# Kmatsuo57/cell-image-analysis

Hardware: NVIDIA B200
Metric: cells scored/sec (crop+resize+CAE+SVM) (higher is better)
Workload: dtype f16 tensor cores (CAE, PCA, SVM cross term: fp16 hi+lo operands, fp32 accumulate) / f64 norms and sums

## Files before the change

cell-image-analysis_b200/csrc/api.cu:

```cuda
#include "common.cuh"

#include <cmath>
#include <cstdlib>
#include <cstring>
#include <new>

#define CIA_VERSION 100

static int bad_handle() { return CIA_E_ARG; }

template <typename T>
static int upload(cia_ctx* h, T** dst, const T* src, size_t n) {
    cudaFree(*dst); *dst = nullptr;
    CIA_CUDA(cudaMalloc((void**)dst, n * sizeof(T)));
    CIA_CUDA(cudaMemcpy(*dst, src, n * sizeof(T), cudaMemcpyHostToDevice));
    return CIA_OK;
}

extern "C" {

int cia_version(void) { return CIA_VERSION; }

void cia_default_params(cia_params* p) {
    if (!p) return;
    p->border_margin = 10;
    p->area_min = 200;
    p->area_max = 8000;
    p->ecc_max = 0.95;
    p->mean_min = 0.5;
    p->std_min = 0.1;
    p->clip_limit = 0.02;
    p->intensity_inv = 1.0 / 65535.0;
}

int cia_create(int device, cia_handle* out) {
    if (!out) return CIA_E_ARG;
    *out = nullptr;
    cia_ctx* h = new (std::nothrow) cia_ctx();
    if (!h) return CIA_E_ARG;
    h->device = device;
    cudaError_t e = cudaSetDevice(device);
    if (e != cudaSuccess) { delete h; return CIA_E_CUDA; }
    cudaDeviceProp prop;
    if (cudaGetDeviceProperties(&prop, device) == cudaSuccess) { h->num_sms = prop.multiProcessorCount; h->max_smem_optin = (int)prop.sharedMemPerBlockOptin; }
    if (cudaMalloc(&h->status_dev, sizeof(int32_t)) != cudaSuccess ||
        cudaMemset(h->status_dev, 0, sizeof(int32_t)) != cudaSuccess ||
        cudaMallocHost(&h->status_host, sizeof(int32_t)) != cudaSuccess ||
        cudaEventCreateWithFlags(&h->ev, cudaEventDisableTiming) != cudaSuccess ||
        cudaEventCreateWithFlags(&h->ev_fork, cudaEventDisableTiming) != cudaSuccess ||
        cudaEventCreateWithFlags(&h->ev_join, cudaEventDisableTiming) != cudaSuccess ||
        cudaStreamCreateWithFlags(&h->side, cudaStreamNonBlocking) != cudaSuccess) {
        delete h;
        return CIA_E_CUDA;
    }
    if (const char* e = getenv("CIA_CAE_CHUNK")) { const int v = atoi(e); if (v > 0) h->cae_pass_cells = v; }
    if (const char* e = getenv("CIA_L1_DEBIAS")) h->cae_debias[0] = (float)atof(e);
    if (const char* e = getenv("CIA_L2_DEBIAS")) h->cae_debias[1] = (float)atof(e);
    if (const char* e = getenv("CIA_L3_DEBIAS")) h->cae_debias[2] = (float)atof(e);
    if (const char* e = getenv("CIA_SVM_KERNEL")) h->svm_kernel = atoi(e) ? 1 : 0;
    if (const char* e = getenv("CIA_PCA_KERNEL")) h->pca_kernel = atoi(e) ? 1 : 0;
    *out = h;
    return CIA_OK;
}

int cia_set_option(cia_handle h, const char* name, double value) {
    if (!h) return bad_handle();
    if (!name) { h->err = "cia_set_option: null name"; return CIA_E_ARG; }
    const std::string n(name);
    if (n == "cae_pass_cells") {
        if (!(value >= 1 && value <= 1 << 20)) { h->err = "cia_set_option: cae_pass_cells must be in [1, 2^20]"; return CIA_E_ARG; }
        h->cae_pass_cells = (int)value;
    } else if (n == "cae_l1_debias" || n == "cae_l2_debias" || n == "cae_l3_debias") {
        if (!(value >= 0 && value <= 64)) { h->err = "cia_set_option: debias must be in [0, 64] (units of 2^-24)"; return CIA_E_ARG; }
        h->cae_debias[n[5] - '1'] = (float)value;
    } else if (n == "svm_kernel") {
        if (value != 0 && value != 1) { h->err = "cia_set_option: svm_kernel is 0 (fp64 DMMA) or 1 (tcgen05)"; return CIA_E_ARG; }
        h->svm_kernel = (int)value;
    } else if (n == "pca_kernel") {
        if (value != 0 && value != 1) { h->err = "cia_set_option: pca_kernel is 0 (fp64 DMMA) or 1 (tcgen05)"; return CIA_E_ARG; }
        h->pca_kernel = (int)value;
    } else if (n == "svm_refine") {
        h->svm_refine = value != 0;
    } else if (n == "seg_conv_tma") {
        h->seg_conv_tma = value != 0;
    } else if (n == "seg_pool_out") {
        h->seg_pool_out = value != 0;
    } else if (n == "seg_fuse_first") {
        h->seg_fuse_first = value != 0;
    } else if (n == "seg_conv_ws") {
        if (value != 0 && value != 1 && value != 2) { h->err = "cia_set_option: seg_conv_ws is 0 (off), 1 (where it pays) or 2 (every layer)"; return CIA_E_ARG; }
        h->seg_conv_ws = (int)value;
    } else {
        h->err = "cia_set_option: unknown option '" + n + "'";
        return CIA_E_ARG;
    }
    return CIA_OK;
}

static void free_cae(CaeWeights& w) {
    for (int i = 0; i < CAE_NCONV; ++i) {
        cudaFree(w.kernel[i]); cudaFree(w.bias[i]); cudaFree(w.bn_scale[i]); cudaFree(w.bn_shift[i]);
        w.kernel[i] = w.bias[i] = w.bn_scale[i] = w.bn_shift[i] = nullptr;
    }
    for (int i = 0; i < CAE_NCONV; ++i)
        for (int j = 0; j < 2; ++j) { cudaFree(w.tc_w[i][j]); w.tc_w[i][j] = nullptr; }
    cudaFree(w.tc_w7); w.tc_w7 = nullptr;
    w.tc_ready = false;
    w.loaded = false;
}

int cia_destroy(cia_handle h) {
    if (!h) return bad_handle();
    cudaSetDevice(h->device);
    cudaDeviceSynchronize();
    free_cae(h->cae[0]); free_cae(h->cae[1]);
    k_seg_free(h);
    cudaFree(h->sp.center); cudaFree(h->sp.scale); cudaFree(h->sp.rscale); cudaFree(h->sp.comp_t); cudaFree(h->sp.comp_pad); cudaFree(h->sp.offset); cudaFree(h->sp.tc_img); cudaFree(h->sp.tc_par);
    for (int i = 0; i < 2; ++i) { cudaFree(h->svm[i].sv_t); cudaFree(h->svm[i].coef); cudaFree(h->svm[i].sv_pad); cudaFree(h->svm[i].gsn);
                                  cudaFree(h->svm[i].tc_hi); cudaFree(h->svm[i].tc_lo); cudaFree(h->svm[i].tc_gcol); }
    Workspace* ws[] = {&h->ws_flags, &h->ws_act, &h->ws_crop_scratch, &h->ws_pipe, &h->ws_feat,
                       &h->ws_misc, &h->ws_stage, &h->ws_svm, &h->ws_fit};
    for (Workspace* w : ws) cudaFree(w->p);
    cudaFree(h->status_dev);
    cudaFreeHost(h->status_host);
    if (h->ev) cudaEventDestroy(h->ev);
    if (h->ev_fork) cudaEventDestroy(h->ev_fork);
    if (h->ev_join) cudaEventDestroy(h->ev_join);
// ... 512 lines not shown
```

cell-image-analysis_b200/csrc/cae_tc.cu:

```cuda
#include "common.cuh"
#include "tc_ptx.cuh"

#include <cuda.h>
#include <cuda_fp16.h>

#include <cmath>

namespace {

constexpr int TCT = 256;
enum { EPI_POOL = 0, EPI_PLAIN = 2, EPI_FINAL = 3, EPI_PHASE = 4 };

using namespace tcptx;

#ifdef CIA_LANE0_ISSUE
#define ISSUE_WARP(cond) (lane == 0 && (cond))
#define ISSUE_BEGIN {
#define ISSUE_END }
#else
#define ISSUE_WARP(cond) (cond)
#define ISSUE_BEGIN if (elect_one()) {
#define ISSUE_END } __syncwarp();
#endif
#ifdef CIA_SPIN_WAIT
// ... 963 lines not shown
                                    fadd2(acc[2 * hp + p2][k8 * 8 + k], acc[2 * hp + p2][k8 * 8 + k + 1],
                                          v[p2][k8][k], v[p2][k8][k + 1]);
                    }
                    DBG_T(e5);
                    DBG_ADD(e_add, e3, e5);
                    ++it;
                }
                DBG_T(e6);
                constexpr int RO = R / 2;
                const int Y = ROWPAIR ? r >> 4 : r >> 3, X = 8 * sub + (r & 7);
#pragma unroll
                for (int k8 = 0; k8 < CW / 8; ++k8) {
                    const int c0 = cq * CW + k8 * 8;
                    float o[8];
#pragma unroll
                    for (int k = 0; k < 8; ++k) {
                        const float b = __ldg(bias + c0 + k), sc = __ldg(bn_s + c0 + k), sh = __ldg(bn_t + c0 + k);
                        float m = acc[0][k8 * 8 + k];
#pragma unroll
                        for (int ph = 1; ph < NT; ++ph) m = fmaxf(m, acc[ph][k8 * 8 + k]);
                        if (ROWPAIR) m = fmaxf(m, __shfl_xor_sync(0xffffffffu, m, 8));
                        o[k] = pooled_act(m, inv_scale, invd, b, sc, sh);
                    }
                    if (ROWPAIR && (r & 8)) continue;
                    const size_t off = ((((size_t)cell * (COUT / 8) + c0 / 8) * RO + Y) * RO + X) * 8;
                    split_store8(o, out_hi + off, out_lo ? out_lo + off : nullptr);
                    if (feat) {
                        float4* f = reinterpret_cast<float4*>(feat + (size_t)cell * (RO * RO * COUT) +
                                                             (size_t)(Y * RO + X) * COUT + c0);
                        f[0] = make_float4(o[0], o[1], o[2], o[3]);
                        f[1] = make_float4(o[4], o[5], o[6], o[7]);
                    }
                }
                DBG_T(e7);
                DBG_ADD(e_final, e6, e7);
            }
        }
#ifdef CIA_ACC_TIMING
        if (tid == 0) {
            atomicAdd(&g_acc_dbg[0], (unsigned long long)e_stage);
            atomicAdd(&g_acc_dbg[1], (unsigned long long)e_full);
            atomicAdd(&g_acc_dbg[2], (unsigned long long)e_ld);
            atomicAdd(&g_acc_dbg[3], (unsigned long long)e_add);
            atomicAdd(&g_acc_dbg[4], (unsigned long long)e_final);
            atomicAdd(&g_acc_dbg[5], (unsigned long long)e_units);
        }
#endif
    }
    tc_fence_before();
    __syncthreads();
    if (warp == 0) tmem_dealloc(tmem_base, TMEM_COLS);
}

template <int G, int VAR = 0>
__global__ void __launch_bounds__(ACC_THREADS, 1)
conv_tc_l2_stack_kernel(const __grid_constant__ CUtensorMap tm_hi, const __grid_constant__ CUtensorMap tm_lo,
                        const uint4* __restrict__ w_hi, const uint4* __restrict__ w_lo, float inv_scale, float invd,
                        const float* __restrict__ bias, const float* __restrict__ bn_s,
                        const float* __restrict__ bn_t, __half* __restrict__ out_hi, __half* __restrict__ out_lo,
                        float* __restrict__ feat, int n_cells, const int32_t* __restrict__ n_dev, int cell0,
                        int chunk_cells) {
    constexpr int CIN = 32, COUT = 64, R = 32;
    using C = Acc2Cfg<CIN, COUT, R>;
    constexpr int NGRP = (9 + G - 1) / G;
    constexpr int CW = COUT / 4;
    constexpr int TILE_COLS = 2 * COUT;
    constexpr int WS_B = 2 * C::W_B;
    extern __shared__ __align__(1024) unsigned char smem[];
    __shared__ __align__(8) uint64_t full_bar[4], empty_bar[4], ready_bar[2];
    __shared__ uint32_t tmem_base_s;

    const int tid = threadIdx.x, warp = tid >> 5, lane = tid & 31;
    unsigned char* const w_s = smem + C::HALVES * C::BUF_B;

    int n = dev_count(n_cells, n_dev) - cell0;
    if (n > chunk_cells) n = chunk_cells;
    if (n <= 0) return;
    const int n_units = n;

    if (warp == 0) tmem_alloc(&tmem_base_s, 512);
    if (tid == 32) {
        for (int t = 0; t < 4; ++t) { mbar_init(&full_bar[t], 1); mbar_init(&empty_bar[t], ACC_EPI_WARPS); }
        mbar_init(&ready_bar[0], 1); mbar_init(&ready_bar[1], 1);
        fence_barrier_init();
    }
    for (int i = tid; i < WS_B / 16; i += ACC_THREADS) {
        const int tc = i / (2 * COUT), row = i - tc * (2 * COUT);
        reinterpret_cast<uint4*>(w_s)[i] = row < COUT ? __ldg(w_hi + tc * COUT + row) : __ldg(w_lo + tc * COUT + row - COUT);
    }
    fence_async_smem();
    tc_fence_before();
    __syncthreads();
    tc_fence_after();
    const uint32_t tmem_base = tmem_base_s;
    const uint32_t sbase = smem_u32(smem);
    constexpr uint32_t IDESC64 = make_idesc(128, COUT), IDESC128 = make_idesc(128, 2 * COUT);

    if (warp >= ACC_EPI_WARPS) {
        if (warp - ACC_EPI_WARPS < 4) {
            const int t = warp - ACC_EPI_WARPS, py = t >> 1, px = t & 1;
            const uint64_t b_s0 = make_smem_desc(smem_u32(w_s), 2 * COUT * 16, 128);
            const uint64_t b_l0 = b_s0 + (uint64_t)((COUT * 16) >> 4);
            uint64_t dxo[3];
#pragma unroll
            for (int dx = 0; dx < 3; ++dx) dxo[dx] = (uint64_t)((((px + dx) & 1) * C::PAR_B + ((px + dx) >> 1) * 16) >> 4);
            const uint32_t d_main = tmem_base + (uint32_t)(t * TILE_COLS), d_cross = d_main + COUT;
// ... 604 lines not shown
                                              w.bn_scale[layer], w.bn_shift[layer], out_hi, out_lo, feat, n, n_dev,
                                              cell0, chunk);
    CIA_LAUNCH_CHECK();
    acc_timing_dump("acc", CIN, COUT, R, G, s);
    return CIA_OK;
}

typedef CUresult (*TensorMapEncodeFn)(CUtensorMap*, CUtensorMapDataType, cuuint32_t, void*, const cuuint64_t*,
                                      const cuuint64_t*, const cuuint32_t*, const cuuint32_t*, CUtensorMapInterleave,
                                      CUtensorMapSwizzle, CUtensorMapL2promotion, CUtensorMapFloatOOBfill);

static int encode_act_map(cia_ctx* h, CUtensorMap* tm, const __half* base, int nch, int r, int cells, int box_x,
                          int box_y) {
    static TensorMapEncodeFn encode = [] {
        void* fn = nullptr;
        cudaDriverEntryPointQueryResult q;
        if (cudaGetDriverEntryPoint("cuTensorMapEncodeTiled", &fn, cudaEnableDefault, &q) != cudaSuccess) fn = nullptr;
        return (TensorMapEncodeFn)fn;
    }();
    if (!encode) { h->err = "cuTensorMapEncodeTiled is not available from this driver"; return CIA_E_UNSUPPORTED; }
    const cuuint64_t dims[5] = {8, (cuuint64_t)r, (cuuint64_t)r, (cuuint64_t)nch, (cuuint64_t)cells};
    const cuuint64_t strides[4] = {16, (cuuint64_t)16 * r, (cuuint64_t)16 * r * r, (cuuint64_t)16 * r * r * nch};
    const cuuint32_t box[5] = {8, (cuuint32_t)box_x, (cuuint32_t)box_y, (cuuint32_t)nch, 1};
    const cuuint32_t estr[5] = {1, 2, 1, 1, 1};
    const CUresult rc = encode(tm, CU_TENSOR_MAP_DATA_TYPE_FLOAT16, 5, (void*)base, dims, strides, box, estr,
                               CU_TENSOR_MAP_INTERLEAVE_NONE, CU_TENSOR_MAP_SWIZZLE_NONE,
                               CU_TENSOR_MAP_L2_PROMOTION_L2_128B, CU_TENSOR_MAP_FLOAT_OOB_FILL_NONE);
    if (rc != CUDA_SUCCESS) { h->err = "cuTensorMapEncodeTiled failed"; return CIA_E_CUDA; }
    return CIA_OK;
}

template <int CIN, int COUT, int R, int G>
int launch_tc_acc2(cia_ctx* h, const CaeWeights& w, int layer, const __half* in_hi, const __half* in_lo,
                   int buf_cells, __half* out_hi, __half* out_lo, float* feat, int n, const int32_t* n_dev,
                   int cell0, int chunk, cudaStream_t s) {
    using C = Acc2Cfg<CIN, COUT, R>;
    static_assert(C::SMEM_B + 1280 <= 227 * 1024, "double-buffered blocks do not fit in shared memory");
    auto kern = conv_tc_acc2_kernel<CIN, COUT, R, G>;
    if (first_use(h, (const void*)kern))
        CIA_CUDA(cudaFuncSetAttribute(kern, cudaFuncAttributeMaxDynamicSharedMemorySize, C::SMEM_B));
    CUtensorMap tm_hi, tm_lo;
    int rc;
    if ((rc = encode_act_map(h, &tm_hi, in_hi, C::NCH, C::R, buf_cells, C::BOX_X, C::FILL_ROWS))) return rc;
    if ((rc = encode_act_map(h, &tm_lo, in_lo, C::NCH, C::R, buf_cells, C::BOX_X, C::FILL_ROWS))) return rc;
    int grid = chunk;
    if (grid > h->num_sms) grid = h->num_sms;
    kern<<<grid, ACC_THREADS, C::SMEM_B, s>>>(tm_hi, tm_lo, (const uint4*)w.tc_w[layer][0],
                                              (const uint4*)w.tc_w[layer][1], w.tc_inv_scale[layer],
                                              w.tc_inv_scale[layer] * acc_debias(h, layer), w.bias[layer],
                                              w.bn_scale[layer], w.bn_shift[layer], out_hi, out_lo, feat, n, n_dev,
                                              cell0, chunk);
    CIA_LAUNCH_CHECK();
    acc_timing_dump("acc2", CIN, COUT, R, G, s);
    return CIA_OK;
}

template <int G, int VAR = 0>
int launch_l2_stack(cia_ctx* h, const CaeWeights& w, const __half* in_hi, const __half* in_lo, int buf_cells,
                    __half* out_hi, __half* out_lo, float* feat, int n, const int32_t* n_dev, int cell0, int chunk,
                    cudaStream_t s) {
    using C = Acc2Cfg<32, 64, 32>;
    auto kern = conv_tc_l2_stack_kernel<G, VAR>;
    if (first_use(h, (const void*)kern))
        CIA_CUDA(cudaFuncSetAttribute(kern, cudaFuncAttributeMaxDynamicSharedMemorySize, C::SMEM_B));
    CUtensorMap tm_hi, tm_lo;
    int rc;
    if ((rc = encode_act_map(h, &tm_hi, in_hi, C::NCH, C::R, buf_cells, C::BOX_X, C::FILL_ROWS))) return rc;
    if ((rc = encode_act_map(h, &tm_lo, in_lo, C::NCH, C::R, buf_cells, C::BOX_X, C::FILL_ROWS))) return rc;
    int grid = chunk;
    if (grid > h->num_sms) grid = h->num_sms;
    kern<<<grid, ACC_THREADS, C::SMEM_B, s>>>(tm_hi, tm_lo, (const uint4*)w.tc_w[1][0], (const uint4*)w.tc_w[1][1],
                                              w.tc_inv_scale[1], w.tc_inv_scale[1] * acc_debias(h, 1), w.bias[1],
                                              w.bn_scale[1], w.bn_shift[1], out_hi, out_lo, feat, n, n_dev, cell0, chunk);
    CIA_LAUNCH_CHECK();
    return CIA_OK;
}

static void pack_image(const std::vector<float>& w , int taps, int cin, int N,
                       int n_real, int sw, std::vector<__half>& hi, std::vector<__half>& lo,
                       const float* colsign = nullptr) {
    const int nch = cin / 8;
    hi.assign((size_t)taps * nch * N * 8, __float2half_rn(0.f));
    lo = hi;
    const float sc = std::ldexp(1.f, sw);
    for (int tap = 0; tap < taps; ++tap)
        for (int c = 0; c < cin; ++c)
            for (int nn = 0; nn < n_real; ++nn) {
                const float v = w[((size_t)tap * cin + c) * n_real + nn] * sc * (colsign ? colsign[nn] : 1.f);
                const __half hv = __float2half_rn(v);
                const size_t idx = (((size_t)tap * nch + c / 8) * N + nn) * 8 + (c % 8);
                hi[idx] = hv;
                lo[idx] = __float2half_rn(v - __half2float(hv));
            }
}

static int scale_exp(const std::vector<float>& w) {
    float m = 0.f;
    for (float v : w) m = std::fmax(m, std::fabs(v));
    if (!(m > 0.f)) return 0;
    int e;
    std::frexp(m, &e);
    return 2 - e;
}

}

// ... 121 lines not shown
        A2f = (float*)h->ws_act.p;
    }
    __half* A1h = (__half*)h->ws_misc.p;
    __half* A1l = A1h + CH * a1;
    __half* A2h = A1l + CH * a1;
    __half* A2l = A2h + CH * a2;
    __half* A3h = A2l + CH * a2;
    __half* A4u = A3h + CH * a3;
    __half* A5u = A4u + CH * a4u;
    __half* A6 = A5u + CH * a5u;
    CIA_CUDA(cudaMemsetAsync(mse, 0, (size_t)n * sizeof(float), s));
    CIA_CUDA(cudaMemsetAsync(mae, 0, (size_t)n * sizeof(float), s));
    const bool side_encoder = features && !tc_feat && !l3_exact;
    if (side_encoder) {
        CIA_CUDA(cudaEventRecord(h->ev_fork, s));
        CIA_CUDA(cudaStreamWaitEvent(h->side, h->ev_fork, 0));
        rc = k_encoder_fp32(h, sep ? h->cae[1] : h->cae[0], crops, n, n_dev, features, h->side);
        if (rc) return rc;
        CIA_CUDA(cudaEventRecord(h->ev_join, h->side));
    }
    for (int c0 = 0; c0 < n; c0 += CH) {
        const int chunk = (n - c0) < CH ? (n - c0) : CH;
        __half* a1h = A1h - (size_t)c0 * a1; __half* a1l = A1l - (size_t)c0 * a1;
        __half* a2h = A2h - (size_t)c0 * a2; __half* a2l = A2l - (size_t)c0 * a2;
        __half* a3h = A3h - (size_t)c0 * a3; __half* a4 = A4u - (size_t)c0 * a4u;
        __half* a5 = A5u - (size_t)c0 * a5u; __half* a6p = A6 - (size_t)c0 * a6;
        float* feat = tc_feat ? features : nullptr;
        int grid1 = chunk * 4;
        if (grid1 > h->num_sms * 8) grid1 = h->num_sms * 8;
        const int pass = c0 / CH;
        if (h->layer_ev && pass < CIA_LAYER_PASSES) h->layer_passes = pass + 1;
#define CIA_LMARK(i) do { if (h->layer_ev && pass < CIA_LAYER_PASSES) CIA_CUDA(cudaEventRecord(h->layer_ev[pass * CIA_LAYER_MARKS + (i)], s)); } while (0)
        CIA_LMARK(0);
        if (tc_feat || l3_exact) {
            static const int l1_tc = [] { const char* e = getenv("CIA_L1_KERNEL"); return e ? atoi(e) : 1; }();
            const float l1_debias = h->cae_debias[0] * 5.9604645e-8f;
            if (l1_tc) {
                if (first_use(h, (const void*)conv1_tc_split_kernel))
                    CIA_CUDA(cudaFuncSetAttribute(conv1_tc_split_kernel, cudaFuncAttributeMaxDynamicSharedMemorySize, l1tc::SMEM_B));
                int gridt = chunk * 8;
                if (gridt > h->num_sms * 2) gridt = h->num_sms * 2;
                conv1_tc_split_kernel<<<gridt, l1tc::NT, l1tc::SMEM_B, s>>>(crops, (const uint4*)ae.tc_w[0][0], ae.tc_inv_scale[0],
                                                                            l1_debias, ae.bias[0], ae.bn_scale[0], ae.bn_shift[0],
                                                                            a1h, a1l, n, n_dev, c0, chunk);
            } else {
                conv1_fp32_planar_kernel<<<grid1, 256, 0, s>>>(crops, ae.kernel[0], ae.bias[0], ae.bn_scale[0],
                                                               ae.bn_shift[0], a1h, a1l, n, n_dev, c0, chunk);
            }
            CIA_LAUNCH_CHECK();
            CIA_LMARK(1);
            float* a2f = l3_exact ? A2f - (size_t)c0 * (16 * 16 * 64) : nullptr;
            static const int l2_g = [] { const char* e = getenv("CIA_L2_TAPS_PER_FLUSH"); return e ? atoi(e) : 3; }();
            static const int l2_stack = [] { const char* e = getenv("CIA_L2_STACK"); return e ? atoi(e) : 0; }();
            if (l2_stack == 2 && l2_g == 3) rc = launch_l2_stack<3, 1>(h, ae, A1h, A1l, CH, a2h, a2l, a2f, n, n_dev, c0, chunk, s);
            else if (l2_stack == 3 && l2_g == 3) rc = launch_l2_stack<3, 2>(h, ae, A1h, A1l, CH, a2h, a2l, a2f, n, n_dev, c0, chunk, s);
            else if (l2_stack && l2_g == 3) rc = launch_l2_stack<3>(h, ae, A1h, A1l, CH, a2h, a2l, a2f, n, n_dev, c0, chunk, s);
            else if (l2_g == 0) rc = launch_tc_acc<32, 64, 32, 1>(h, ae, 1, a1h, a1l, a2h, a2l, a2f, n, n_dev, c0, chunk, s);
            else if (l2_g == 1) rc = launch_tc_acc2<32, 64, 32, 1>(h, ae, 1, A1h, A1l, CH, a2h, a2l, a2f, n, n_dev, c0, chunk, s);
            else if (l2_g == 9) rc = launch_tc_acc2<32, 64, 32, 9>(h, ae, 1, A1h, A1l, CH, a2h, a2l, a2f, n, n_dev, c0, chunk, s);
            else if (l2_g == 2) rc = launch_tc_acc2<32, 64, 32, 2>(h, ae, 1, A1h, A1l, CH, a2h, a2l, a2f, n, n_dev, c0, chunk, s);
            else rc = launch_tc_acc2<32, 64, 32, 3>(h, ae, 1, A1h, A1l, CH, a2h, a2l, a2f, n, n_dev, c0, chunk, s);
            if (rc) return rc;
            CIA_LMARK(2);
            if (l3_exact) {
                if ((rc = launch_tc<64, 32, 16, EPI_POOL, 1>(h, ae, 2, a2h, nullptr, a3h, nullptr, nullptr, nullptr, nullptr, nullptr, n, n_dev, c0, chunk, s))) return rc;
                if (features && (rc = k_conv3_fp32(h, ae, a2f, n, n_dev, features, c0, chunk, s))) return rc;
            } else {
                static const int l3_tma = [] { const char* e = getenv("CIA_L3_KERNEL"); return e ? atoi(e) : 0; }();
                static const int l3_g = [] { const char* e = getenv("CIA_L3_TAPS_PER_FLUSH"); return e ? atoi(e) : 1; }();
                if (l3_tma) rc = launch_tc_acc2<64, 32, 16, 1>(h, ae, 2, A2h, A2l, CH, a3h, nullptr, feat, n, n_dev, c0, chunk, s);
                else if (l3_g == 3) rc = launch_tc_acc<64, 32, 16, 3>(h, ae, 2, a2h, a2l, a3h, nullptr, feat, n, n_dev, c0, chunk, s);
                else rc = launch_tc_acc<64, 32, 16, 1>(h, ae, 2, a2h, a2l, a3h, nullptr, feat, n, n_dev, c0, chunk, s);
                if (rc) return rc;
            }
        } else {
            conv1_fp32_planar_kernel<<<grid1, 256, 0, s>>>(crops, ae.kernel[0], ae.bias[0], ae.bn_scale[0],
                                                           ae.bn_shift[0], a1h, nullptr, n, n_dev, c0, chunk);
            CIA_LAUNCH_CHECK();
            CIA_LMARK(1);
            if ((rc = launch_tc<32, 64, 32, EPI_POOL, 1>(h, ae, 1, a1h, nullptr, a2h, nullptr, nullptr, nullptr, nullptr, nullptr, n, n_dev, c0, chunk, s))) return rc;
            CIA_LMARK(2);
            if ((rc = launch_tc<64, 32, 16, EPI_POOL, 1>(h, ae, 2, a2h, nullptr, a3h, nullptr, nullptr, nullptr, nullptr, nullptr, n, n_dev, c0, chunk, s))) return rc;
        }
        CIA_LMARK(3);
        if ((rc = launch_tc<32, 32, 8, EPI_PLAIN, 1>(h, ae, 3, a3h, nullptr, a4, nullptr, nullptr, nullptr, nullptr, nullptr, n, n_dev, c0, chunk, s))) return rc;
        CIA_LMARK(4);
        if ((rc = launch_tc<32, 64, 16, EPI_PLAIN, 1, true>(h, ae, 4, a4, nullptr, a5, nullptr, nullptr, nullptr, nullptr, nullptr, n, n_dev, c0, chunk, s))) return rc;
        CIA_LMARK(5);
        if ((rc = launch_tc<64, 128, 16, EPI_PHASE, 1>(h, ae, 5, a5, nullptr, a6p, nullptr, nullptr, nullptr, nullptr, nullptr, n, n_dev, c0, chunk, s))) return rc;
        CIA_LMARK(6);
        static const int l7_tapsum = [] { const char* e = getenv("CIA_L7_KERNEL"); return e ? atoi(e) : 1; }();
        if (l7_tapsum) {
            if (first_use(h, (const void*)final_tapsum_kernel))
                CIA_CUDA(cudaFuncSetAttribute(final_tapsum_kernel, cudaFuncAttributeMaxDynamicSharedMemorySize, l7::SMEM_B));
            int g7 = chunk < h->num_sms ? chunk : h->num_sms;
            final_tapsum_kernel<<<g7, l7::NT, l7::SMEM_B, s>>>(a6p, (const uint4*)ae.tc_w7, ae.tc_inv_scale[6], ae.bias[6],
                                                              crops, mse, mae, n, n_dev, c0, chunk);
            CIA_LAUNCH_CHECK();
        } else if ((rc = launch_tc<32, 16, 32, EPI_FINAL, 1>(h, ae, 6, a6p, nullptr, nullptr, nullptr, nullptr, crops, mse, mae, n, n_dev, c0, chunk, s))) return rc;
        CIA_LMARK(7);
#undef CIA_LMARK
    }
    if (side_encoder) CIA_CUDA(cudaStreamWaitEvent(s, h->ev_join, 0));
    return CIA_OK;
}
```

cell-image-analysis_b200/csrc/common.cuh:

```cuda
#pragma once
#include <cuda_runtime.h>
#include <stdint.h>
#include <stdio.h>
#include <set>
#include <string>
#include <vector>

#include "../../include/cia.h"

#define CIA_NUM_SMS_DEFAULT 148

#define CAE_NCONV 7
static const int kCaeCin[CAE_NCONV]  = {1, 32, 64, 32, 32, 64, 32};
static const int kCaeCout[CAE_NCONV] = {32, 64, 32, 32, 64, 32, 1};

struct CaeWeights {
    bool loaded = false;
    int n_conv = 0;
    float* kernel[CAE_NCONV] = {};
    float* bias[CAE_NCONV] = {};
    float* bn_scale[CAE_NCONV] = {};
    float* bn_shift[CAE_NCONV] = {};
    void* tc_w[CAE_NCONV][2] = {};
    void* tc_w7 = nullptr;
// ... 19 lines not shown

struct ScalerPca {
    bool loaded = false;
    int F = 0, C = 0;
    int center_is_f32 = 1, f32_flow = 1, has_center = 0, has_scale = 0;
    double* center = nullptr;
    double* scale = nullptr;
    double* rscale = nullptr;
    bool rscale_ok = false;
    double* comp_t = nullptr;
    double* comp_pad = nullptr;
    int CP = 0;
    double* offset = nullptr;
    void* tc_img = nullptr;
    void* tc_par = nullptr;
    int tc_ew = 0;
    bool tc_ok = false;
};

struct Workspace {
    void* p = nullptr;
    size_t cap = 0;
};

struct SegModel;

struct cia_ctx {
    int device = 0;
    SegModel* seg = nullptr;
    int num_sms = CIA_NUM_SMS_DEFAULT;
    int max_smem_optin = 227 * 1024;
    std::string err;
    CaeWeights cae[2];
    ScalerPca sp;
    SvmModel svm[2];
    int32_t* status_dev = nullptr;
    int32_t* status_host = nullptr;
    int64_t launches = 0;
    std::set<const void*> attr_done;
    Workspace ws_flags, ws_act, ws_crop_scratch, ws_pipe, ws_feat, ws_misc, ws_stage, ws_svm;
    Workspace ws_fit;
    cudaEvent_t ev = nullptr;
    cudaStream_t side = nullptr;
    cudaEvent_t ev_fork = nullptr, ev_join = nullptr;
    std::vector<cudaEvent_t> prof_ev;
    std::vector<cudaEvent_t> prof_layer_ev;
    std::vector<int> prof_layer_passes;
    int layer_passes = 0;
    cudaEvent_t* layer_ev = nullptr;
    bool prof_layers_valid = false;
    int prof_records = 0, prof_used = 0;
    int cae_pass_cells = 18944;
    float cae_debias[3] = {0.5f, 2.4f, 1.2f};
    int svm_kernel = 1;
    int pca_kernel = 1;
    int seg_fuse_first = 0;
    int seg_pool_out = 1;
    int seg_conv_ws = 1;
    int seg_conv_tma = 1;
    int svm_refine = 1;
};
#define CIA_LAYER_MARKS 8
#define CIA_LAYER_PASSES 8
#define CIA_PROF_MARKS 7

#define CIA_CUDA(call)                                                              \
    do {                                                                            \
        cudaError_t e_ = (call);                                                    \
        if (e_ != cudaSuccess) {                                                    \
            h->err = std::string(#call) + ": " + cudaGetErrorString(e_);            \
            return CIA_E_CUDA;                                                      \
        }                                                                           \
    } while (0)

#define CIA_LAUNCH_CHECK()                                                          \
    do {                                                                            \
        h->launches++;                                                              \
        cudaError_t e_ = cudaGetLastError();                                        \
        if (e_ != cudaSuccess) {                                                    \
            h->err = std::string("kernel launch: ") + cudaGetErrorString(e_);       \
            return CIA_E_CUDA;                                                      \
        }                                                                           \
    } while (0)

static inline int ws_reserve(cia_ctx* h, Workspace& w, size_t bytes) {
    if (bytes <= w.cap) return CIA_OK;
    if (w.p) {
        CIA_CUDA(cudaDeviceSynchronize());
        CIA_CUDA(cudaFree(w.p));
        w.p = nullptr; w.cap = 0;
    }
    size_t want = bytes + bytes / 4 + 256;
    CIA_CUDA(cudaMalloc(&w.p, want));
    w.cap = want;
    return CIA_OK;
}

static inline bool first_use(cia_ctx* h, const void* fn) { return h->attr_done.insert(fn).second; }

__device__ __forceinline__ int dev_count(int n, const int32_t* n_dev) {
    if (n_dev == nullptr) return n;
    int m = *n_dev;
    return m < n ? m : n;
}

__device__ __forceinline__ void raise_status(int32_t* status, int code) {
// ... 63 lines not shown
```

cell-image-analysis_b200/csrc/tc_ptx.cuh:

```cuda
#pragma once
#include <cuda_runtime.h>
#include <stdint.h>

namespace tcptx {

__device__ __forceinline__ uint32_t smem_u32(const void* p) { return (uint32_t)__cvta_generic_to_shared(p); }

__device__ __forceinline__ void mbar_init(uint64_t* bar, uint32_t count) {
    asm volatile("mbarrier.init.shared::cta.b64 [%0], %1;" ::"r"(smem_u32(bar)), "r"(count) : "memory");
}
__device__ __forceinline__ void mbar_wait(uint64_t* bar, uint32_t parity) {
    const uint32_t a = smem_u32(bar);
    uint32_t done;
    do {
        asm volatile(
            "{\n\t.reg .pred p;\n\t"
            "mbarrier.try_wait.parity.shared::cta.b64 p, [%1], %2;\n\t"
            "selp.u32 %0, 1, 0, p;\n\t}"
            : "=r"(done) : "r"(a), "r"(parity) : "memory");
    } while (!done);
}
__device__ __forceinline__ void mbar_wait_sleep(uint64_t* bar, uint32_t parity) {
    const uint32_t a = smem_u32(bar);
    asm volatile(
// ... 20 lines not shown
    asm volatile("tcgen05.relinquish_alloc_permit.cta_group::1.sync.aligned;" ::: "memory");
}
__device__ __forceinline__ void tmem_dealloc(uint32_t taddr, uint32_t ncols) {
    asm volatile("tcgen05.dealloc.cta_group::1.sync.aligned.b32 %0, %1;" ::"r"(taddr), "r"(ncols) : "memory");
}
__device__ __forceinline__ void umma_f16(uint32_t d_tmem, uint64_t adesc, uint64_t bdesc, uint32_t idesc,
                                         uint32_t accumulate) {
    asm volatile(
        "{\n\t.reg .pred p;\n\tsetp.ne.b32 p, %4, 0;\n\t"
        "tcgen05.mma.cta_group::1.kind::f16 [%0], %1, %2, %3, p;\n\t}"
        ::"r"(d_tmem), "l"(adesc), "l"(bdesc), "r"(idesc), "r"(accumulate) : "memory");
}
__device__ __forceinline__ void umma_commit(uint64_t* bar) {
    asm volatile("tcgen05.commit.cta_group::1.mbarrier::arrive::one.shared::cluster.b64 [%0];" ::"r"(smem_u32(bar)) : "memory");
}
#define TMEM_LD8(taddr, v)                                                                          \
    asm volatile("tcgen05.ld.sync.aligned.32x32b.x8.b32 {%0,%1,%2,%3,%4,%5,%6,%7}, [%8];"            \
                 : "=r"(v[0]), "=r"(v[1]), "=r"(v[2]), "=r"(v[3]), "=r"(v[4]), "=r"(v[5]), "=r"(v[6]), \
                   "=r"(v[7]) : "r"(taddr))
#define TMEM_WAIT8(v)                                                                               \
    asm volatile("tcgen05.wait::ld.sync.aligned;"                                                   \
                 : "+r"(v[0]), "+r"(v[1]), "+r"(v[2]), "+r"(v[3]), "+r"(v[4]), "+r"(v[5]), "+r"(v[6]), \
                   "+r"(v[7]) :: "memory")

#define TMEM_LD16(taddr, v)                                                                               \
    asm volatile("tcgen05.ld.sync.aligned.32x32b.x16.b32 "                                                \
                 "{%0,%1,%2,%3,%4,%5,%6,%7,%8,%9,%10,%11,%12,%13,%14,%15}, [%16];"                         \
                 : "=r"(v[0]), "=r"(v[1]), "=r"(v[2]), "=r"(v[3]), "=r"(v[4]), "=r"(v[5]), "=r"(v[6]),     \
                   "=r"(v[7]), "=r"(v[8]), "=r"(v[9]), "=r"(v[10]), "=r"(v[11]), "=r"(v[12]), "=r"(v[13]), \
                   "=r"(v[14]), "=r"(v[15]) : "r"(taddr))
#define TMEM_WAIT16(v)                                                                                    \
    asm volatile("tcgen05.wait::ld.sync.aligned;"                                                         \
                 : "+r"(v[0]), "+r"(v[1]), "+r"(v[2]), "+r"(v[3]), "+r"(v[4]), "+r"(v[5]), "+r"(v[6]),     \
                   "+r"(v[7]), "+r"(v[8]), "+r"(v[9]), "+r"(v[10]), "+r"(v[11]), "+r"(v[12]), "+r"(v[13]), \
                   "+r"(v[14]), "+r"(v[15]) :: "memory")

__device__ __forceinline__ uint64_t make_smem_desc(uint32_t saddr, uint32_t lbo_bytes, uint32_t sbo_bytes) {
    uint64_t d = 0;
    d |= (uint64_t)((saddr >> 4) & 0x3FFFu);
    d |= (uint64_t)((lbo_bytes >> 4) & 0x3FFFu) << 16;
    d |= (uint64_t)((sbo_bytes >> 4) & 0x3FFFu) << 32;
    d |= (uint64_t)1 << 46;
    return d;
}
__host__ __device__ constexpr uint32_t make_idesc(int M, int N) {
    return (1u << 4) | ((uint32_t)(N >> 3) << 17) | ((uint32_t)(M >> 4) << 24);
}
__host__ __device__ constexpr int pow2_cols(int c) { return c <= 32 ? 32 : c <= 64 ? 64 : c <= 128 ? 128 : c <= 256 ? 256 : 512; }

__device__ __forceinline__ void mbar_arrive(uint64_t* bar) {
    asm volatile("mbarrier.arrive.shared::cta.b64 _, [%0];" ::"r"(smem_u32(bar)) : "memory");
}

__device__ __forceinline__ void mbar_expect_tx(uint64_t* bar, uint32_t bytes) {
    asm volatile("mbarrier.arrive.expect_tx.shared::cta.b64 _, [%0], %1;" ::"r"(smem_u32(bar)), "r"(bytes) : "memory");
}
__device__ __forceinline__ void bulk_load(uint32_t dst, const void* src, uint32_t bytes, uint64_t* bar) {
    asm volatile("cp.async.bulk.shared::cluster.global.mbarrier::complete_tx::bytes [%0], [%1], %2, [%3];"
                 ::"r"(dst), "l"(src), "r"(bytes), "r"(smem_u32(bar)) : "memory");
}


__device__ __forceinline__ unsigned long long pack2(float lo, float hi) {
    unsigned long long r;
    asm("mov.b64 %0, {%1,%2};" : "=l"(r) : "f"(lo), "f"(hi));
    return r;
}
__device__ __forceinline__ void unpack2(unsigned long long v, float& lo, float& hi) {
    asm("mov.b64 {%0,%1}, %2;" : "=f"(lo), "=f"(hi) : "l"(v));
}
__device__ __forceinline__ unsigned long long fma2(unsigned long long a, unsigned long long b, unsigned long long c) {
    unsigned long long d;
    asm("fma.rn.f32x2 %0, %1, %2, %3;" : "=l"(d) : "l"(a), "l"(b), "l"(c));
    return d;
}
__device__ __forceinline__ void fadd2(float& a0, float& a1, uint32_t b0, uint32_t b1) {
    asm("{\n\t.reg .b64 ra, rb;\n\tmov.b64 ra, {%0,%1};\n\tmov.b64 rb, {%2,%3};\n\t"
        "add.rn.f32x2 ra, ra, rb;\n\tmov.b64 {%0,%1}, ra;\n\t}"
        : "+f"(a0), "+f"(a1) : "r"(b0), "r"(b1));
}


}
```

Measured before the change: 3.155 million.

## Add CTA-pair tcgen05 conv kernel for CAE layer 3 using 2-SM UMMA

```diff
diff --git a/cell-image-analysis_b200/csrc/api.cu b/cell-image-analysis_b200/csrc/api.cu
--- a/cell-image-analysis_b200/csrc/api.cu
+++ b/cell-image-analysis_b200/csrc/api.cu
@@ -57,6 +57,7 @@
     if (const char* e = getenv("CIA_L1_DEBIAS")) h->cae_debias[0] = (float)atof(e);
     if (const char* e = getenv("CIA_L2_DEBIAS")) h->cae_debias[1] = (float)atof(e);
     if (const char* e = getenv("CIA_L3_DEBIAS")) h->cae_debias[2] = (float)atof(e);
+    if (const char* e = getenv("CIA_L3_PAIR")) h->cae_l3_pair = atoi(e) ? 1 : 0;
     if (const char* e = getenv("CIA_SVM_KERNEL")) h->svm_kernel = atoi(e) ? 1 : 0;
     if (const char* e = getenv("CIA_PCA_KERNEL")) h->pca_kernel = atoi(e) ? 1 : 0;
     *out = h;
@@ -73,6 +74,9 @@
     } else if (n == "cae_l1_debias" || n == "cae_l2_debias" || n == "cae_l3_debias") {
         if (!(value >= 0 && value <= 64)) { h->err = "cia_set_option: debias must be in [0, 64] (units of 2^-24)"; return CIA_E_ARG; }
         h->cae_debias[n[5] - '1'] = (float)value;
+    } else if (n == "cae_l3_pair") {
+        if (value != 0 && value != 1) { h->err = "cia_set_option: cae_l3_pair is 0 (single-CTA kernel) or 1 (CTA pairs)"; return CIA_E_ARG; }
+        h->cae_l3_pair = (int)value;
     } else if (n == "svm_kernel") {
         if (value != 0 && value != 1) { h->err = "cia_set_option: svm_kernel is 0 (fp64 DMMA) or 1 (tcgen05)"; return CIA_E_ARG; }
         h->svm_kernel = (int)value;
diff --git a/cell-image-analysis_b200/csrc/cae_tc.cu b/cell-image-analysis_b200/csrc/cae_tc.cu
--- a/cell-image-analysis_b200/csrc/cae_tc.cu
+++ b/cell-image-analysis_b200/csrc/cae_tc.cu
@@ -1039,6 +1039,246 @@
     if (warp == 0) tmem_dealloc(tmem_base, TMEM_COLS);
 }
 
+template <int CIN, int COUT, int R>
+struct PairCfg {
+    using A = Acc2Cfg<CIN, COUT, R>;
+    static constexpr bool STACK = A::ROWPAIR && COUT <= 32;
+    static constexpr int TC = 9 * A::NCH;
+    static constexpr int WA_N = STACK ? COUT : COUT / 2;
+    static constexpr int WB_N = COUT / 2;
+    static constexpr int WA_B = TC * WA_N * 16;
+    static constexpr int WB_B = TC * WB_N * 16;
+    static constexpr int SMEM_B = 2 * A::BUF_B + WA_B + WB_B;
+};
+
+template <int CIN, int COUT, int R, int G, int NST_ = 0>
+__global__ void __launch_bounds__(ACC_THREADS, 1)
+conv_tc_acc2_pair_kernel(const __grid_constant__ CUtensorMap tm_hi, const __grid_constant__ CUtensorMap tm_lo,
+                         const uint4* __restrict__ w_hi, const uint4* __restrict__ w_lo, float inv_scale, float invd,
+                         const float* __restrict__ bias, const float* __restrict__ bn_s,
+                         const float* __restrict__ bn_t, __half* __restrict__ out_hi, __half* __restrict__ out_lo,
+                         float* __restrict__ feat, int n_cells, const int32_t* __restrict__ n_dev, int cell0,
+                         int chunk_cells) {
+    using C = Acc2Cfg<CIN, COUT, R>;
+    using P = PairCfg<CIN, COUT, R>;
+    constexpr bool ROWPAIR = C::ROWPAIR, STACK = P::STACK;
+    constexpr int NT = ROWPAIR ? 2 : 4;
+    constexpr int TILE_COLS = STACK ? 2 * COUT : COUT;
+    constexpr int STAGE_COLS = NT * TILE_COLS;
+    constexpr int NST = NST_ > 0 ? NST_ : (4 * STAGE_COLS <= 512 ? 4 : 2);
+    constexpr int TMEM_COLS = pow2_cols(NST * STAGE_COLS);
+    constexpr int CW = COUT / 4;
+    constexpr int NGRP = (9 + G - 1) / G;
+    extern __shared__ __align__(1024) unsigned char smem[];
+    __shared__ __align__(8) uint64_t full_bar[NST], empty_bar[NST], ready_bar[2];
+    __shared__ uint32_t tmem_base_s;
+
+    const int tid = threadIdx.x, warp = tid >> 5, lane = tid & 31;
+    const uint32_t rank = cluster_rank();
+    const int pair = blockIdx.x >> 1, npairs = gridDim.x >> 1;
+    unsigned char* wa = smem + 2 * C::BUF_B;
+    unsigned char* wb = wa + P::WA_B;
+
+    int n = dev_count(n_cells, n_dev) - cell0;
+    if (n > chunk_cells) n = chunk_cells;
+    if (n <= 0) return;
+    const int n_units = (n + 1) >> 1;
+    const int n_blocks = pair < n_units ? (n_units - 1 - pair) / npairs * C::HALVES + C::HALVES : 0;
+    const uint32_t sbase = smem_u32(smem);
+    auto load_block = [&](int b) {
+        if (b >= n_blocks) return;
+        const int cell_rel = 2 * (pair + b / C::HALVES * npairs) + (int)rank;
+        tma_load_half_block<C>(&tm_hi, &tm_lo, sbase + (b & 1) * C::BUF_B, cell_rel < n ? cell_rel : cell_rel - 1,
+                               b % C::HALVES, &ready_bar[b & 1]);
+    };
+
+    if (warp == 0) tmem_alloc_pair(&tmem_base_s, TMEM_COLS);
+    if (tid == 32) {
+        for (int i = 0; i < NST; ++i) { mbar_init(&full_bar[i], NT); mbar_init(&empty_bar[i], 2 * ACC_EPI_WARPS); }
+        mbar_init(&ready_bar[0], rank == 0 ? 2 : 1); mbar_init(&ready_bar[1], rank == 0 ? 2 : 1);
+        fence_barrier_init();
+    }
+    for (int i = tid; i < P::WA_B / 16; i += ACC_THREADS) {
+        const int tc = i / P::WA_N, row = i - tc * P::WA_N;
+        reinterpret_cast<uint4*>(wa)[i] = __ldg((STACK && rank ? w_lo : w_hi) + tc * COUT + (STACK ? 0 : (int)rank * P::WA_N) + row);
+    }
+    for (int i = tid; i < P::WB_B / 16; i += ACC_THREADS) {
+        const int tc = i / P::WB_N, row = i - tc * P::WB_N;
+        reinterpret_cast<uint4*>(wb)[i] = __ldg((STACK ? w_hi : w_lo) + tc * COUT + (int)rank * P::WB_N + row);
+    }
+    fence_async_smem();
+    tc_fence_before();
+    cluster_sync();
+    tc_fence_after();
+    const uint32_t tmem_base = tmem_base_s;
+
+    if (warp >= ACC_EPI_WARPS) {
+        if (rank == 0) {
+            if (ISSUE_WARP(warp - ACC_EPI_WARPS < NT)) {
+                const int t = warp - ACC_EPI_WARPS, py = ROWPAIR ? 0 : t >> 1, px = t & 1;
+                const uint64_t b_a0 = make_smem_desc(smem_u32(wa), P::WA_N * 16, 128);
+                const uint64_t b_b0 = make_smem_desc(smem_u32(wb), P::WB_N * 16, 128);
+                constexpr uint32_t IDESC = make_idesc(256, COUT), IDESC2 = make_idesc(256, TILE_COLS);
+                uint64_t dxo[3];
+#pragma unroll
+                for (int dx = 0; dx < 3; ++dx) dxo[dx] = (uint64_t)((((px + dx) & 1) * C::PAR_B + ((px + dx) >> 1) * 16) >> 4);
+                uint32_t it = 0;
+                for (int b = 0; b < n_blocks; ++b) {
+                    const uint32_t abase = sbase + (b & 1) * C::BUF_B + py * C::ROW_B;
+                    const uint64_t a_hi0 = make_smem_desc(abase, C::PLANE_B, C::SBO_A);
+                    const uint64_t a_lo0 = make_smem_desc(abase + C::REGION_B, C::PLANE_B, C::SBO_A);
+                    MBAR_WAIT(&ready_bar[b & 1], (b >> 1) & 1);
+                    tc_fence_after();
+#pragma unroll
+                    for (int grp = 0; grp < NGRP; ++grp) {
+                        const uint32_t st = it % NST;
+                        MBAR_WAIT(&empty_bar[st], ((it / NST) & 1) ^ 1);
+                        tc_fence_after();
+                        const uint32_t d = tmem_base + st * STAGE_COLS + (uint32_t)(t * TILE_COLS);
+                        ISSUE_BEGIN
+                        if (STACK) {
+#pragma unroll
+                            for (int pass = 0; pass < 2; ++pass) {
+#pragma unroll
+                                for (int tg = 0; tg < G; ++tg) {
+                                    const int tap = grp * G + tg;
+                                    if (tap < 9) {
+                                        const int dy = tap / 3, dx = tap % 3;
+                                        const uint64_t a0 = (pass == 1 ? a_lo0 : a_hi0) + dxo[dx];
+#pragma unroll
+                                        for (int s = 0; s < CIN / 16; ++s) {
+                                            const uint64_t ad = a0 + (uint64_t)((dy * C::ROW_B + 2 * s * C::PLANE_B) >> 4);
+                                            const int tcs = tap * C::NCH + 2 * s;
+                                            if (pass == 0) umma_f16_pair(d, ad, b_a0 + (uint64_t)((tcs * P::WA_N * 16) >> 4), IDESC2,
+                                                                         (tg == 0 && s == 0) ? 0u : 1u);
+                                            else umma_f16_pair(d + COUT, ad, b_b0 + (uint64_t)((tcs * P::WB_N * 16) >> 4), IDESC, 1u);
+                                        }
+                                    }
+                                }
+                            }
+                        } else
+#pragma unroll
+                        for (int pass = 0; pass < 3; ++pass) {
+#pragma unroll
+                            for (int tg = 0; tg < G; ++tg) {
+                                const int tap = grp * G + tg;
+                                if (tap < 9) {
+                                    const int dy = tap / 3, dx = tap % 3;
+                                    const uint64_t a0 = (pass == 1 ? a_lo0 : a_hi0) + dxo[dx];
+                                    const uint64_t b0 = pass == 0 ? b_b0 : b_a0;
+#pragma unroll
+                                    for (int s = 0; s < CIN / 16; ++s) {
+                                        const uint64_t ad = a0 + (uint64_t)((dy * C::ROW_B + 2 * s * C::PLANE_B) >> 4);
+                                        const uint64_t bd = b0 + (uint64_t)((((tap * C::NCH + 2 * s) * P::WB_N) * 16) >> 4);
+                                        umma_f16_pair(d, ad, bd, IDESC, (pass == 0 && tg == 0 && s == 0) ? 0u : 1u);
+                                    }
+                                }
+                            }
+                        }
+                        umma_commit_pair(&full_bar[st]);
+                        ISSUE_END
+                        ++it;
+                    }
+                }
+            }
+        } else if (warp == ACC_EPI_WARPS) {
+            for (int b = 0; b < n_blocks; ++b) {
+                MBAR_WAIT(&ready_bar[b & 1], (b >> 1) & 1);
+                if (lane == 0) mbar_arrive_cluster(&ready_bar[b & 1], 0);
+                __syncwarp();
+            }
+        }
+    } else {
+        const int q = warp & 3, cq = warp >> 2;
+        const int r = 32 * q + lane;
+        const uint32_t lane_addr = tmem_base + ((uint32_t)(32 * q) << 16) + (uint32_t)(cq * CW);
+        uint32_t it = 0;
+        if (tid == 0) { load_block(0); load_block(1); }
+        for (int b = 0; b < n_blocks; ++b) {
+            const int sub = b % C::HALVES;
+            const int cell_rel = 2 * (pair + b / C::HALVES * npairs) + (int)rank;
+            const int cell = cell0 + cell_rel;
+            float acc[NT][CW];
+#pragma unroll
+            for (int ph = 0; ph < NT; ++ph)
+#pragma unroll
+                for (int k = 0; k < CW; ++k) acc[ph][k] = 0.f;
+#pragma unroll 1
+            for (int grp = 0; grp < NGRP; ++grp) {
+                const uint32_t st = it % NST;
+                MBAR_WAIT(&full_bar[st], (it / NST) & 1);
+                tc_fence_after();
+                if (grp == NGRP - 1 && tid == 0) load_block(b + 2);
+#pragma unroll
+                for (int hp = 0; hp < NT / 2; ++hp) {
+                    uint32_t v[2][CW / 8][8];
+                    uint32_t vc[2][STACK ? CW / 8 : 1][8];
+#pragma unroll
+                    for (int p2 = 0; p2 < 2; ++p2)
+#pragma unroll
+                        for (int k8 = 0; k8 < CW / 8; ++k8) {
+                            TMEM_LD8(lane_addr + st * STAGE_COLS + (uint32_t)((2 * hp + p2) * TILE_COLS + k8 * 8), v[p2][k8]);
+                            if (STACK) TMEM_LD8(lane_addr + st * STAGE_COLS + (uint32_t)((2 * hp + p2) * TILE_COLS + COUT + k8 * 8), vc[p2][k8]);
+                        }
+#pragma unroll
+                    for (int p2 = 0; p2 < 2; ++p2)
+#pragma unroll
+                        for (int k8 = 0; k8 < CW / 8; ++k8) {
+                            TMEM_WAIT8(v[p2][k8]);
+                            if (STACK) TMEM_WAIT8(vc[p2][k8]);
+                        }
+                    if (hp == NT / 2 - 1) {
+                        tc_fence_before();
+                        __syncwarp();
+                        if (lane == 0) mbar_arrive_cluster(&empty_bar[st], 0);
+                    }
+#pragma unroll
+                    for (int p2 = 0; p2 < 2; ++p2)
+#pragma unroll
+                        for (int k8 = 0; k8 < CW / 8; ++k8)
+#pragma unroll
+                            for (int k = 0; k < 8; k += 2) {
+                                if (STACK) fadd2(acc[2 * hp + p2][k8 * 8 + k], acc[2 * hp + p2][k8 * 8 + k + 1],
+                                                 vc[p2][k8][k], vc[p2][k8][k + 1]);
+                                fadd2(acc[2 * hp + p2][k8 * 8 + k], acc[2 * hp + p2][k8 * 8 + k + 1],
+                                      v[p2][k8][k], v[p2][k8][k + 1]);
+                            }
+                }
+                ++it;
+            }
+            constexpr int RO = R / 2;
+            const int Y = ROWPAIR ? r >> 4 : r >> 3, X = 8 * sub + (r & 7);
+#pragma unroll
+            for (int k8 = 0; k8 < CW / 8; ++k8) {
+                const int c0 = cq * CW + k8 * 8;
+                float o[8];
+#pragma unroll
+                for (int k = 0; k < 8; ++k) {
+                    const float bb = __ldg(bias + c0 + k), sc = __ldg(bn_s + c0 + k), sh = __ldg(bn_t + c0 + k);
+                    float m = acc[0][k8 * 8 + k];
+#pragma unroll
+                    for (int ph = 1; ph < NT; ++ph) m = fmaxf(m, acc[ph][k8 * 8 + k]);
+                    if (ROWPAIR) m = fmaxf(m, __shfl_xor_sync(0xffffffffu, m, 8));
+                    o[k] = pooled_act(m, inv_scale, invd, bb, sc, sh);
+                }
+                if (cell_rel >= n) continue;
+                if (ROWPAIR && (r & 8)) continue;
+                const size_t off = ((((size_t)cell * (COUT / 8) + c0 / 8) * RO + Y) * RO + X) * 8;
+                split_store8(o, out_hi + off, out_lo ? out_lo + off : nullptr);
+                if (feat) {
+                    float4* f = reinterpret_cast<float4*>(feat + (size_t)cell * (RO * RO * COUT) +
+                                                         (size_t)(Y * RO + X) * COUT + c0);
+                    f[0] = make_float4(o[0], o[1], o[2], o[3]);
+                    f[1] = make_float4(o[4], o[5], o[6], o[7]);
+                }
+            }
+        }
+    }
+    tc_fence_before();
+    cluster_sync();
+    if (warp == 0) tmem_dealloc_pair(tmem_base, TMEM_COLS);
+}
+
 template <int G, int VAR = 0>
 __global__ void __launch_bounds__(ACC_THREADS, 1)
 conv_tc_l2_stack_kernel(const __grid_constant__ CUtensorMap tm_hi, const __grid_constant__ CUtensorMap tm_lo,
@@ -1749,6 +1989,49 @@
                                               cell0, chunk);
     CIA_LAUNCH_CHECK();
     acc_timing_dump("acc2", CIN, COUT, R, G, s);
+    return CIA_OK;
+}
+
+template <int CIN, int COUT, int R, int G, int NST = 0>
+int launch_tc_acc2_pair(cia_ctx* h, const CaeWeights& w, int layer, const __half* in_hi, const __half* in_lo,
+                        int buf_cells, __half* out_hi, __half* out_lo, float* feat, int n, const int32_t* n_dev,
+                        int cell0, int chunk, cudaStream_t s) {
+    using C = Acc2Cfg<CIN, COUT, R>;
+    using P = PairCfg<CIN, COUT, R>;
+    static_assert(P::SMEM_B + 1280 <= 227 * 1024, "double-buffered blocks do not fit in shared memory");
+    auto kern = conv_tc_acc2_pair_kernel<CIN, COUT, R, G, NST>;
+    if (first_use(h, (const void*)kern))
+        CIA_CUDA(cudaFuncSetAttribute(kern, cudaFuncAttributeMaxDynamicSharedMemorySize, P::SMEM_B));
+    CUtensorMap tm_hi, tm_lo;
+    int rc;
+    if ((rc = encode_act_map(h, &tm_hi, in_hi, C::NCH, C::R, buf_cells, C::BOX_X, C::FILL_ROWS))) return rc;
+    if ((rc = encode_act_map(h, &tm_lo, in_lo, C::NCH, C::R, buf_cells, C::BOX_X, C::FILL_ROWS))) return rc;
+    cudaLaunchAttribute attr[1];
+    attr[0].id = cudaLaunchAttributeClusterDimension;
+    attr[0].val.clusterDim.x = 2;
+    attr[0].val.clusterDim.y = 1;
+    attr[0].val.clusterDim.z = 1;
+    cudaLaunchConfig_t cfg = {};
+    cfg.blockDim = dim3(ACC_THREADS);
+    cfg.dynamicSmemBytes = P::SMEM_B;
+    cfg.stream = s;
+    cfg.attrs = attr;
+    cfg.numAttrs = 1;
+    static const int resident = [&] {
+        int c = 0;
+        cfg.gridDim = dim3(h->num_sms & ~1);
+        if (cudaOccupancyMaxActiveClusters(&c, kern, &cfg) != cudaSuccess || c <= 0) { cudaGetLastError(); c = h->num_sms / 2; }
+        if (getenv("CIA_PAIR_DEBUG")) fprintf(stderr, "pair kernel: %d resident clusters\n", c);
+        return c;
+    }();
+    int pairs = (chunk + 1) / 2;
+    if (pairs > resident) pairs = resident;
+    cfg.gridDim = dim3(2 * pairs);
+    CIA_CUDA(cudaLaunchKernelEx(&cfg, kern, tm_hi, tm_lo, (const uint4*)w.tc_w[layer][0], (const uint4*)w.tc_w[layer][1],
+                                w.tc_inv_scale[layer], w.tc_inv_scale[layer] * acc_debias(h, layer),
+                                (const float*)w.bias[layer], (const float*)w.bn_scale[layer], (const float*)w.bn_shift[layer],
+                                out_hi, out_lo, feat, n, n_dev, cell0, chunk));
+    CIA_LAUNCH_CHECK();
     return CIA_OK;
 }
 
@@ -1976,7 +2259,9 @@
             float* a2f = l3_exact ? A2f - (size_t)c0 * (16 * 16 * 64) : nullptr;
             static const int l2_g = [] { const char* e = getenv("CIA_L2_TAPS_PER_FLUSH"); return e ? atoi(e) : 3; }();
             static const int l2_stack = [] { const char* e = getenv("CIA_L2_STACK"); return e ? atoi(e) : 0; }();
-            if (l2_stack == 2 && l2_g == 3) rc = launch_l2_stack<3, 1>(h, ae, A1h, A1l, CH, a2h, a2l, a2f, n, n_dev, c0, chunk, s);
+            static const int l2_pair = [] { const char* e = getenv("CIA_L2_PAIR"); return e ? atoi(e) : 0; }();
+            if (l2_pair && l2_g == 3) rc = launch_tc_acc2_pair<32, 64, 32, 3>(h, ae, 1, A1h, A1l, CH, a2h, a2l, a2f, n, n_dev, c0, chunk, s);
+            else if (l2_stack == 2 && l2_g == 3) rc = launch_l2_stack<3, 1>(h, ae, A1h, A1l, CH, a2h, a2l, a2f, n, n_dev, c0, chunk, s);
             else if (l2_stack == 3 && l2_g == 3) rc = launch_l2_stack<3, 2>(h, ae, A1h, A1l, CH, a2h, a2l, a2f, n, n_dev, c0, chunk, s);
             else if (l2_stack && l2_g == 3) rc = launch_l2_stack<3>(h, ae, A1h, A1l, CH, a2h, a2l, a2f, n, n_dev, c0, chunk, s);
             else if (l2_g == 0) rc = launch_tc_acc<32, 64, 32, 1>(h, ae, 1, a1h, a1l, a2h, a2l, a2f, n, n_dev, c0, chunk, s);
@@ -1992,7 +2277,12 @@
             } else {
                 static const int l3_tma = [] { const char* e = getenv("CIA_L3_KERNEL"); return e ? atoi(e) : 0; }();
                 static const int l3_g = [] { const char* e = getenv("CIA_L3_TAPS_PER_FLUSH"); return e ? atoi(e) : 1; }();
-                if (l3_tma) rc = launch_tc_acc2<64, 32, 16, 1>(h, ae, 2, A2h, A2l, CH, a3h, nullptr, feat, n, n_dev, c0, chunk, s);
+                static const int l3_nst = [] { const char* e = getenv("CIA_L3_PAIR_STAGES"); return e ? atoi(e) : 0; }();
+                if (h->cae_l3_pair && !l3_tma && l3_g == 1 && l3_nst == 2)
+                    rc = launch_tc_acc2_pair<64, 32, 16, 1, 2>(h, ae, 2, A2h, A2l, CH, a3h, nullptr, feat, n, n_dev, c0, chunk, s);
+                else if (h->cae_l3_pair && !l3_tma && l3_g == 1)
+                    rc = launch_tc_acc2_pair<64, 32, 16, 1>(h, ae, 2, A2h, A2l, CH, a3h, nullptr, feat, n, n_dev, c0, chunk, s);
+                else if (l3_tma) rc = launch_tc_acc2<64, 32, 16, 1>(h, ae, 2, A2h, A2l, CH, a3h, nullptr, feat, n, n_dev, c0, chunk, s);
                 else if (l3_g == 3) rc = launch_tc_acc<64, 32, 16, 3>(h, ae, 2, a2h, a2l, a3h, nullptr, feat, n, n_dev, c0, chunk, s);
                 else rc = launch_tc_acc<64, 32, 16, 1>(h, ae, 2, a2h, a2l, a3h, nullptr, feat, n, n_dev, c0, chunk, s);
                 if (rc) return rc;
diff --git a/cell-image-analysis_b200/csrc/common.cuh b/cell-image-analysis_b200/csrc/common.cuh
--- a/cell-image-analysis_b200/csrc/common.cuh
+++ b/cell-image-analysis_b200/csrc/common.cuh
@@ -95,6 +95,7 @@
     int prof_records = 0, prof_used = 0;
     int cae_pass_cells = 18944;
     float cae_debias[3] = {0.5f, 2.4f, 1.2f};
+    int cae_l3_pair = 1;
     int svm_kernel = 1;
     int pca_kernel = 1;
     int seg_fuse_first = 0;
diff --git a/cell-image-analysis_b200/csrc/tc_ptx.cuh b/cell-image-analysis_b200/csrc/tc_ptx.cuh
--- a/cell-image-analysis_b200/csrc/tc_ptx.cuh
+++ b/cell-image-analysis_b200/csrc/tc_ptx.cuh
@@ -96,6 +96,39 @@
     asm volatile("mbarrier.arrive.shared::cta.b64 _, [%0];" ::"r"(smem_u32(bar)) : "memory");
 }
 
+__device__ __forceinline__ uint32_t cluster_rank() {
+    uint32_t r;
+    asm volatile("mov.u32 %0, %%cluster_ctarank;" : "=r"(r));
+    return r;
+}
+__device__ __forceinline__ void cluster_sync() {
+    asm volatile("barrier.cluster.arrive.release.aligned;\n\tbarrier.cluster.wait.acquire.aligned;" ::: "memory");
+}
+__device__ __forceinline__ void tmem_alloc_pair(uint32_t* dst_smem, uint32_t ncols) {
+    asm volatile("tcgen05.alloc.cta_group::2.sync.aligned.shared::cta.b32 [%0], %1;" ::"r"(smem_u32(dst_smem)), "r"(ncols) : "memory");
+    asm volatile("tcgen05.relinquish_alloc_permit.cta_group::2.sync.aligned;" ::: "memory");
+}
+__device__ __forceinline__ void tmem_dealloc_pair(uint32_t taddr, uint32_t ncols) {
+    asm volatile("tcgen05.dealloc.cta_group::2.sync.aligned.b32 %0, %1;" ::"r"(taddr), "r"(ncols) : "memory");
+}
+__device__ __forceinline__ void umma_f16_pair(uint32_t d_tmem, uint64_t adesc, uint64_t bdesc, uint32_t idesc,
+                                              uint32_t accumulate) {
+    asm volatile(
+        "{\n\t.reg .pred p;\n\tsetp.ne.b32 p, %4, 0;\n\t"
+        "tcgen05.mma.cta_group::2.kind::f16 [%0], %1, %2, %3, p;\n\t}"
+        ::"r"(d_tmem), "l"(adesc), "l"(bdesc), "r"(idesc), "r"(accumulate) : "memory");
+}
+__device__ __forceinline__ void umma_commit_pair(uint64_t* bar) {
+    asm volatile("tcgen05.commit.cta_group::2.mbarrier::arrive::one.shared::cluster.multicast::cluster.b64 [%0], %1;"
+                 ::"r"(smem_u32(bar)), "h"((uint16_t)0x3) : "memory");
+}
+__device__ __forceinline__ void mbar_arrive_cluster(uint64_t* bar, uint32_t rank) {
+    asm volatile(
+        "{\n\t.reg .b32 ra;\n\tmapa.shared::cluster.u32 ra, %0, %1;\n\t"
+        "mbarrier.arrive.shared::cluster.b64 _, [ra];\n\t}"
+        ::"r"(smem_u32(bar)), "r"(rank) : "memory");
+}
+
 __device__ __forceinline__ void mbar_expect_tx(uint64_t* bar, uint32_t bytes) {
     asm volatile("mbarrier.arrive.expect_tx.shared::cta.b64 _, [%0], %1;" ::"r"(smem_u32(bar)), "r"(bytes) : "memory");
 }
```

After: 3.237 million (median of 6 runs). +2.6%, better.
